# barathanaslan/whisper-ipa

Measured on AMD Instinct MI355X. Metric: audio-seconds/sec transcribed (whisper-small, 30s clips), higher is better.
Workload: dtype bf16

## Files before the change

### include/wipa.h

```cpp
#ifndef WIPA_H
#define WIPA_H
#include <stddef.h>
#include <stdint.h>
#ifdef __cplusplus
extern "C" {
#endif

typedef void* wipa_stream_t;

enum { WIPA_F32 = 0, WIPA_BF16 = 1, WIPA_FP8_E4M3 = 2  };
enum { WIPA_OK = 0, WIPA_ERR_ARG = -1, WIPA_ERR_HIP = -2, WIPA_ERR_STATE = -3 };

#define WIPA_N_SAMPLES 480000
#define WIPA_N_FRAMES 3000
#define WIPA_N_FFT 400
#define WIPA_HOP 160
#define WIPA_HEAD_DIM 64

int wipa_version(void);
const char* wipa_last_error(void);

int wipa_stream_create(wipa_stream_t* out);
int wipa_stream_create_cu_limited(int n_cus, wipa_stream_t* out);
int wipa_stream_destroy(wipa_stream_t s);
// ... 76 lines not shown
                   const float* b, int rows, int D, float eps, wipa_stream_t s);

int wipa_layernorm_fp8(const float* x, int64_t ldx, void* y, int64_t ldy, float* y_scale, const float* w, const float* b, int rows,
                       int D, float eps, wipa_stream_t s);
int wipa_rowquant_fp8(const void* x, int x_dtype, int64_t ldx, void* y, int64_t ldy, float* y_scale, int rows, int D, wipa_stream_t s);

int wipa_add_slabs_layernorm(float* x, int64_t ldx, const float* slabs, int n_slabs, int64_t slab_stride, void* y,
                             int y_dtype, int64_t ldy, const float* w, const float* b, int rows, int D, float eps,
                             wipa_stream_t s);

int wipa_embed_tokens(const int32_t* tokens, int64_t ld_tok, int B, int T, int t_start, const int32_t* pos_dev,
                      const void* tok_emb, int emb_dtype, const float* emb_scale, const float* pos_emb, float* x, int D,
                      wipa_stream_t s);

typedef struct wipa_attn_desc {
    const void* q;
    const void* k;
    const void* v;
    void* out;
    const int32_t* tk_dev;
    const int32_t* q_row_dev;
    float* lse;
    int64_t q_bs, q_rs, q_hs;
    int64_t k_bs, k_rs, k_hs;
    int64_t v_bs, v_rs, v_hs;
    int64_t o_bs, o_rs, o_hs;
    int32_t B, H, Tq, Tk;
    int32_t causal, dtype;
} wipa_attn_desc;
int wipa_attention(const wipa_attn_desc* d, wipa_stream_t s);

int wipa_flash_attn_enc_bf16(const void* qk, int64_t ldqk, const void* vt, int64_t ldvt, void* out, int64_t ldo,
                             int B, int H, int T, wipa_stream_t s);
int wipa_flash_attn_enc_f32(const float* q, int64_t ldq, const float* k, int64_t ldk, const float* v, int64_t ldv, float* out,
                            int64_t ldo, int B, int H, int T, int f32_split, wipa_stream_t s);

int wipa_decode_attn(const wipa_attn_desc* d, wipa_stream_t s);
int wipa_decode_cross_attn(const void* q, const void* kv, void* out, int B, int H, int Tk, int dtype,
                           wipa_stream_t s);
int wipa_decode_cross_attn_multi(const void* q, const void* kv, void* out, int B, int H, int Tk, int n_q, int dtype,
                                 wipa_stream_t s);

int wipa_decode_cross_attn_grouped(const void* q, const void* kv, void* out, int B, int H, int Tk, int n_q, int n_group, int dtype,
                                   wipa_stream_t s);

typedef struct wipa_self_block_desc {
    const float* x;
    const float* ln_w;
    const float* ln_b;
    const void* wqkv;
    const float* bqkv;
    const void* wo;
    void* kcache;
    void* vcache;
    const int32_t* pos;
    float* slabs;
    int64_t kv_batch_stride, slab_stride;
    int32_t B, d, H, dtype;
    float eps, qk_scale;
} wipa_self_block_desc;
int wipa_decode_self_block(const wipa_self_block_desc* d, wipa_stream_t s);
typedef struct wipa_cross_block_desc {
    const float* x_in;
    float* x_out;
    const float* slabs;
    const float* bias_o;
// ... 298 lines not shown
```

### whisper_ipa_amd/_lib.py

```python
from __future__ import annotations

import ctypes as C
import os
import threading

_HERE = os.path.dirname(os.path.abspath(__file__))
LIB_PATH = os.path.join(_HERE, "libwipa.so")

WIPA_F32, WIPA_BF16, WIPA_FP8_E4M3 = 0, 1, 2
GREEDY_PARTS = 2048
RESAMPLE_TILE = 512
SCORE_MAX_LEN = 1024
ENC_GLOBAL, ENC_PER_LAYER = 7, 14
DEC_GLOBAL, DEC_PER_LAYER, DEC_FP8_PER_LAYER = 4, 20, 6
GEMM_DISPATCH = ("tile128", "tile256", "tile384", "tile384n", "tile256p", "skinny", "skinny_fp8", "skinny_ln", "kmajor", "split_k",
                 "tile_fp8", "tile_fp8_384")
ENC_FP8_PER_LAYER = 8
DEC_ABSORBED_PER_LAYER = 1

c_void_p, c_int, c_int64, c_size_t, c_float = C.c_void_p, C.c_int, C.c_int64, C.c_size_t, C.c_float


class GemmDesc(C.Structure):
    _fields_ = [
# ... 67 lines not shown
    _fields_ = [(n, c_int64) for n in (
        "total_bytes", "tokens", "ld_tok", "pos", "not_done", "sum_logprobs", "logits", "ld_logits",
        "cross_kv", "self_kv", "scratch")]


_P = C.POINTER
SIGNATURES = {
    "wipa_version": (c_int, []),
    "wipa_last_error": (C.c_char_p, []),
    "wipa_stream_create": (c_int, [C.POINTER(c_void_p)]),
    "wipa_stream_create_cu_limited": (c_int, [c_int, C.POINTER(c_void_p)]),
    "wipa_stream_destroy": (c_int, [c_void_p]),
    "wipa_resample_pad": (c_int, [c_void_p, c_size_t, c_void_p, _P(PcmClipDesc), c_int, c_void_p, c_size_t, c_void_p, c_void_p]),
    "wipa_logmel_tables_bytes": (c_size_t, [c_int]),
    "wipa_logmel_init": (c_int, [c_void_p, c_int, c_void_p]),
    "wipa_logmel_workspace_bytes": (c_size_t, [c_int, c_int]),
    "wipa_logmel": (c_int, [c_void_p, c_int, c_int, c_void_p, c_void_p, c_int, c_void_p, c_size_t, c_void_p]),
    "wipa_mel_pad_cast": (c_int, [c_void_p, c_int, c_int, c_void_p, c_int, c_void_p]),
    "wipa_gemm": (c_int, [_P(GemmDesc), c_void_p]),
    "wipa_gemm_dispatch_counts": (c_int, [_P(c_int64), c_int, c_int]),
    "wipa_layernorm": (c_int, [c_void_p, c_int, c_int64, c_void_p, c_int, c_int64, c_void_p, c_void_p, c_int, c_int,
                               c_float, c_void_p]),
    "wipa_layernorm_fp8": (c_int, [c_void_p, c_int64, c_void_p, c_int64, c_void_p, c_void_p, c_void_p, c_int, c_int, c_float, c_void_p]),
    "wipa_rowquant_fp8": (c_int, [c_void_p, c_int, c_int64, c_void_p, c_int64, c_void_p, c_int, c_int, c_void_p]),
    "wipa_add_slabs_layernorm": (c_int, [c_void_p, c_int64, c_void_p, c_int, c_int64, c_void_p, c_int, c_int64, c_void_p,
                                         c_void_p, c_int, c_int, c_float, c_void_p]),
    "wipa_embed_tokens": (c_int, [c_void_p, c_int64, c_int, c_int, c_int, c_void_p, c_void_p, c_int, c_void_p, c_void_p, c_void_p,
                                  c_int, c_void_p]),
    "wipa_attention": (c_int, [_P(AttnDesc), c_void_p]),
    "wipa_flash_attn_enc_f32": (c_int, [c_void_p, c_int64, c_void_p, c_int64, c_void_p, c_int64, c_void_p, c_int64, c_int, c_int,
                                       c_int, c_int, c_void_p]),
    "wipa_flash_attn_enc_bf16": (c_int, [c_void_p, c_int64, c_void_p, c_int64, c_void_p, c_int64, c_int, c_int, c_int,
                                         c_void_p]),
    "wipa_decode_attn": (c_int, [_P(AttnDesc), c_void_p]),
    "wipa_decode_cross_attn": (c_int, [c_void_p, c_void_p, c_void_p, c_int, c_int, c_int, c_int, c_void_p]),
    "wipa_decode_self_block": (c_int, [_P(SelfBlockDesc), c_void_p]),
    "wipa_decode_cross_block": (c_int, [_P(CrossBlockDesc), c_void_p]),
    "wipa_cross_absorbed_splits": (c_int, [c_int, c_int]),
    "wipa_cross_absorbed_resident_groups_for": (c_int, [c_int, c_int, c_int, c_int, c_int64]),
    "wipa_cross_absorbed_resident_groups": (c_int, [c_int, c_int, c_int, c_int]),
    "wipa_cross_absorbed_scratch_bytes": (c_size_t, [c_int, c_int, c_int]),
    "wipa_cross_absorbed_init": (c_int, [c_int]),
    "wipa_cross_absorbed_attention": (c_int, [c_void_p, c_int64, c_void_p, c_void_p, c_void_p, c_void_p, c_void_p, c_int64, c_void_p, c_size_t,
                                              c_int, c_int, c_int, c_int, c_float, c_int, c_void_p]),
    "wipa_cross_absorbed_stream": (c_int, [c_void_p, c_void_p, c_size_t, c_int, c_int, c_int, c_int, c_int, c_void_p]),
    "wipa_decode_cross_absorbed_block": (c_int, [_P(CrossBlockDesc), c_void_p, c_void_p, c_void_p, c_void_p, c_size_t, c_void_p]),
    "wipa_decode_cross_absorbed_block_out": (c_int, [_P(CrossBlockDesc), c_void_p, c_void_p, c_void_p, c_void_p, c_void_p, c_void_p, c_int64,
                                                     c_void_p, c_size_t, c_void_p]),
    "wipa_greedy_step": (c_int, [c_void_p, c_int64, c_int, c_int, c_void_p, c_void_p, c_void_p, c_int64, c_void_p, c_int,
                                 c_int, c_void_p, c_void_p, c_void_p]),
    "wipa_add_i32": (c_int, [c_void_p, C.c_int32, c_void_p]),
    "wipa_greedy_step_embed": (c_int, [c_void_p, c_int64, c_int, c_int, c_void_p, c_void_p, c_void_p, c_int64, c_void_p, c_void_p, c_void_p,
                                       c_int, c_int, c_void_p, c_void_p, c_void_p, c_int, c_void_p, c_void_p, c_int, c_void_p, c_void_p,
                                       c_void_p, c_void_p, c_int, c_int, c_float, c_void_p]),
    "wipa_timestamp_step": (c_int, [c_void_p, c_int64, c_int, c_int, c_void_p, c_void_p, c_void_p, c_int64, c_void_p, c_int, c_int,
                                    _P(DecodeRules), c_void_p, c_void_p, c_void_p]),
    "wipa_timestamp_step_embed": (c_int, [c_void_p, c_int64, c_int, c_int, c_void_p, c_void_p, c_void_p, c_int64, c_void_p, c_void_p, c_void_p,
                                          c_int, c_int, _P(DecodeRules), c_void_p, c_void_p, c_void_p, c_int, c_void_p, c_void_p, c_int,
                                          c_void_p, c_void_p, c_void_p, c_void_p, c_int, c_int, c_float, c_void_p]),
    "wipa_sample_record_bytes": (c_size_t, [c_int]),
    "wipa_sample_record_fill": (c_int, [c_void_p, c_size_t, C.c_uint64, c_int, c_float, c_void_p, c_int]),
    "wipa_sample_step": (c_int, [c_void_p, c_int64, c_int, c_int, c_void_p, c_void_p, c_void_p, c_int64, c_void_p, c_int, c_int,
                                 _P(DecodeRules), c_void_p, c_void_p, c_void_p, c_void_p]),
    "wipa_sample_step_embed": (c_int, [c_void_p, c_int64, c_int, c_int, c_void_p, c_void_p, c_void_p, c_int64, c_void_p, c_void_p, c_void_p,
                                       c_int, c_int, _P(DecodeRules), c_void_p, c_void_p, c_void_p, c_void_p, c_int, c_void_p, c_void_p, c_int,
                                       c_void_p, c_void_p, c_void_p, c_void_p, c_int, c_int, c_float, c_void_p]),
# ... 155 lines not shown
```

### whisper_ipa_amd/csrc/attention.hip

```cpp
#include <cstring>

#include "attn_stream.h"
#include "wipa_common.h"

namespace {

struct AttnParams {
    const char* q;
    const char* k;
    const char* v;
    char* out;
    const int32_t* tk_dev;
    const int32_t* q_row_dev;
    float* lse;
    int64_t q_bs, q_rs, q_hs, k_bs, k_rs, k_hs, v_bs, v_rs, v_hs, o_bs, o_rs, o_hs;
    int Tq, Tk, causal, H;
};

template <bool RAGGED, bool GROUPED = false, bool BEAM = false>
struct AttnArgs : AttnParams {};
template <>
struct AttnArgs<true> : AttnParams {
    const int32_t* k_start;
};
// ... 383 lines not shown
                    const int key = kt * 64 + 32 * u + (i & 3) + 8 * (i >> 2) + 4 * hh;            \
                    if (key >= T) S[u][i] = NEG_BIG;                                               \
                }                                                                                  \
        }                                                                                          \
        float mx = NEG_BIG;                                                                        \
        _Pragma("unroll") for (int u = 0; u < 2; ++u)                                              \
            _Pragma("unroll") for (int i = 0; i < 16; ++i) mx = fmaxf(mx, S[u][i]);                \
        mx = fmaxf(mx, __shfl_xor(mx, 32, 64));                                                    \
        const float m_new = fmaxf(m, mx * LOG2E);                                                  \
        f32x2 psum2 = {0.f, 0.f};                                                                  \
        const f32x2 l2e = {LOG2E, LOG2E}, mneg = {-m_new, -m_new};                                 \
        _Pragma("unroll") for (int u = 0; u < 2; ++u)                                              \
            _Pragma("unroll") for (int i = 0; i < 16; i += 2) {                                    \
                const f32x2 x = __builtin_elementwise_fma(f32x2{S[u][i], S[u][i + 1]}, l2e, mneg); \
                const f32x2 pv = {__builtin_amdgcn_exp2f(x.x), __builtin_amdgcn_exp2f(x.y)};       \
                S[u][i] = pv.x;                                                                    \
                S[u][i + 1] = pv.y;                                                                \
                psum2 += pv;                                                                       \
            }                                                                                      \
        const float psum = psum2.x + psum2.y;                                                      \
        if (__any(m_new > m)) {                                                                    \
            const float alpha = __builtin_amdgcn_exp2f(m - m_new);                                 \
            l *= alpha;                                                                            \
            _Pragma("unroll") for (int i = 0; i < 16; ++i) {                                       \
                O[0][i] *= alpha;                                                                  \
                O[1][i] *= alpha;                                                                  \
            }                                                                                      \
            m = m_new;                                                                             \
        }                                                                                          \
        l += psum;                                                                                 \
    } while (0)
#define WIPA_FLASH_SOFTMAX_FINISH() l += __shfl_xor(l, 32, 64)

__global__ __launch_bounds__(512) void flash_enc_bf16_kernel(const __bf16* __restrict__ qk, int64_t ldqk,
                                                             const __bf16* __restrict__ vt, int64_t ldvt,
                                                             __bf16* __restrict__ out, int64_t ldo, int H, int T) {
    __shared__ __attribute__((aligned(16))) char smem[4 * FA_TILE];
    const int tid = threadIdx.x, lane = tid & 63, wave = tid >> 6;
    const int r = lane & 31, hh = lane >> 5;
    const int h = blockIdx.y, b = blockIdx.z;
    const int D = H * 64;
    const int nw = blockDim.x >> 6;
    const int q0 = blockIdx.x * (nw * 32) + wave * 32;
    const int nkt = (T + 63) / 64;

    bf16x8 qf[4];
    {
        const int qrow = min(q0 + r, T - 1);
        const __bf16* qp = qk + ((int64_t)b * T + qrow) * ldqk + h * 64 + 8 * hh;
#pragma unroll
        for (int s = 0; s < 4; ++s) qf[s] = *reinterpret_cast<const bf16x8*>(qp + 16 * s);
    }
    typedef __attribute__((address_space(3))) void* lds_t;
    const __bf16* kbase = qk + (int64_t)b * T * ldqk + D + h * 64;
    const __bf16* vbase = vt + ((int64_t)b * D + h * 64) * ldvt;
    const __amdgpu_buffer_rsrc_t rK = __builtin_amdgcn_make_buffer_rsrc((void*)kbase, 0, (int)(((int64_t)(T - 1) * ldqk + 64) * 2), 0x00020000);
    const __amdgpu_buffer_rsrc_t rV = __builtin_amdgcn_make_buffer_rsrc((void*)vbase, 0, (int)(((int64_t)63 * ldvt + ldvt) * 2), 0x00020000);
    const int wv = __builtin_amdgcn_readfirstlane(wave);
    const int ppw = 8 / nw;
    int offK[2], offV[2];
#pragma unroll
    for (int i = 0; i < 2; ++i) {
        const int row = 8 * (ppw * wv + i) + (lane >> 3);
        const int c = (lane & 7) ^ ((row >> 1) & 7);
        offK[i] = row * (int)ldqk * 2 + c * 16;
        offV[i] = row * (int)ldvt * 2 + c * 16;
    }
    auto stage = [&](int kt, int buf) {
        char* base = smem + buf * 2 * FA_TILE + (ppw * wv) * 1024;
        const int k0 = kt * 64;
#pragma unroll
        for (int i = 0; i < 2; ++i) {
            if (i < ppw) {
                __builtin_amdgcn_raw_ptr_buffer_load_lds(rK, (lds_t)(base + i * 1024), 16, offK[i], k0 * (int)ldqk * 2, 0, 0);
                __builtin_amdgcn_raw_ptr_buffer_load_lds(rV, (lds_t)(base + FA_TILE + i * 1024), 16, offV[i], k0 * 2, 0, 0);
            }
        }
    };

    f32x16 O[2];
#pragma unroll
    for (int i = 0; i < 16; ++i) O[0][i] = O[1][i] = 0.f;
    float m = NEG_BIG, l = 0.f;
    const int rsw = (r >> 1) & 7;

    stage(0, 0);
    asm volatile("s_waitcnt vmcnt(0)" ::: "memory");
    __syncthreads();
    for (int kt = 0; kt < nkt; ++kt) {
        if (kt + 1 < nkt) stage(kt + 1, (kt + 1) & 1);
        const char* kbuf = smem + (kt & 1) * 2 * FA_TILE;
        const char* vbuf = kbuf + FA_TILE;
        f32x16 S[2];
#pragma unroll
        for (int u = 0; u < 2; ++u) {
#pragma unroll
            for (int i = 0; i < 16; ++i) S[u][i] = 0.f;
            const char* krow = kbuf + (32 * u + r) * FA_ROWB;
#pragma unroll
            for (int s = 0; s < 4; ++s) {
                const bf16x8 kf = *reinterpret_cast<const bf16x8*>(krow + (((2 * s + hh) ^ rsw) << 4));
                S[u] = __builtin_amdgcn_mfma_f32_32x32x16_bf16(kf, qf[s], S[u], 0, 0, 0);
            }
        }
        WIPA_FLASH_SOFTMAX_TILE();
#pragma unroll
        for (int u = 0; u < 2; ++u)
#pragma unroll
            for (int sp = 0; sp < 2; ++sp) {
                bf16x8 pb;
#pragma unroll
                for (int j = 0; j < 8; ++j) pb[j] = (__bf16)S[u][8 * sp + j];
#pragma unroll
                for (int dt = 0; dt < 2; ++dt) {
                    const char* vrow = vbuf + (32 * dt + r) * FA_ROWB + 8 * hh;
                    const int c0 = 4 * u + 2 * sp;
                    const bf16x4 lo = *reinterpret_cast<const bf16x4*>(vrow + ((c0 ^ rsw) << 4));
                    const bf16x4 hi = *reinterpret_cast<const bf16x4*>(vrow + (((c0 + 1) ^ rsw) << 4));
                    const bf16x8 vf = {lo[0], lo[1], lo[2], lo[3], hi[0], hi[1], hi[2], hi[3]};
                    O[dt] = __builtin_amdgcn_mfma_f32_32x32x16_bf16(vf, pb, O[dt], 0, 0, 0);
                    asm volatile("" ::: "memory");
                }
            }
        asm volatile("s_waitcnt vmcnt(0)" ::: "memory");
        __syncthreads();
    }
    WIPA_FLASH_SOFTMAX_FINISH();
    const int qrow = q0 + r;
    if (qrow < T) {
        const float inv = 1.f / l;
        __bf16* op = out + ((int64_t)b * T + qrow) * ldo + h * 64 + 4 * hh;
#pragma unroll
        for (int dt = 0; dt < 2; ++dt)
#pragma unroll
            for (int g4 = 0; g4 < 4; ++g4) {
                bf16x4 o = {(__bf16)(O[dt][4 * g4] * inv), (__bf16)(O[dt][4 * g4 + 1] * inv),
                            (__bf16)(O[dt][4 * g4 + 2] * inv), (__bf16)(O[dt][4 * g4 + 3] * inv)};
                *reinterpret_cast<bf16x4*>(op + 32 * dt + 8 * g4) = o;
            }
    }
}

constexpr int FF_LD = 68;
constexpr int FF_TILE = 64 * FF_LD;

__device__ __forceinline__ void stage_k_parity(float* krow, int kseg, const f32x4 (&rk)[4]) {
    float* kt = krow + 8 * kseg;
    *reinterpret_cast<f32x4*>(kt) = f32x4{rk[0][0], rk[0][2], rk[1][0], rk[1][2]};
    *reinterpret_cast<f32x4*>(kt + 4) = f32x4{rk[2][0], rk[2][2], rk[3][0], rk[3][2]};
    *reinterpret_cast<f32x4*>(kt + 32) = f32x4{rk[0][1], rk[0][3], rk[1][1], rk[1][3]};
    *reinterpret_cast<f32x4*>(kt + 36) = f32x4{rk[2][1], rk[2][3], rk[3][1], rk[3][3]};
}
__device__ __forceinline__ void stage_k_plain(float* krow, int kseg, const f32x4 (&rk)[4]) {
    float* kt = krow + 16 * kseg;
#pragma unroll
    for (int c = 0; c < 4; ++c) *reinterpret_cast<f32x4*>(kt + 4 * c) = rk[c];
// ... 132 lines not shown
                S[u] = __builtin_amdgcn_mfma_f32_32x32x16_bf16(kh, qh[s], S[u], 0, 0, 0);
            }
        }
        WIPA_FLASH_SOFTMAX_TILE();
#pragma unroll
        for (int u = 0; u < 2; ++u)
#pragma unroll
            for (int sp = 0; sp < 2; ++sp) {
                bf16x8 ph, pl;
                split_bf16x2(f32x4{S[u][8 * sp], S[u][8 * sp + 1], S[u][8 * sp + 2], S[u][8 * sp + 3]},
                             f32x4{S[u][8 * sp + 4], S[u][8 * sp + 5], S[u][8 * sp + 6], S[u][8 * sp + 7]}, ph, pl);
#pragma unroll
                for (int dt = 0; dt < 2; ++dt) {
                    const float* vr = vbuf + (32 * dt + r) * FF_LD + 32 * u + 16 * sp + 4 * hh;
                    bf16x8 vh, vl;
                    split_bf16x2(*reinterpret_cast<const f32x4*>(vr), *reinterpret_cast<const f32x4*>(vr + 8), vh, vl);
                    O[dt] = __builtin_amdgcn_mfma_f32_32x32x16_bf16(vh, pl, O[dt], 0, 0, 0);
                    O[dt] = __builtin_amdgcn_mfma_f32_32x32x16_bf16(vl, ph, O[dt], 0, 0, 0);
                    O[dt] = __builtin_amdgcn_mfma_f32_32x32x16_bf16(vh, ph, O[dt], 0, 0, 0);
                }
            }
        WIPA_FLASH_F32_TILE_END();
    }
    WIPA_FLASH_F32_TAIL();
}

#undef WIPA_FLASH_F32_INDICES
#undef WIPA_FLASH_F32_STAGING
#undef WIPA_FLASH_F32_TILE_BEGIN
#undef WIPA_FLASH_F32_TILE_END
#undef WIPA_FLASH_F32_TAIL
#undef WIPA_FLASH_SOFTMAX_TILE
#undef WIPA_FLASH_SOFTMAX_FINISH

}

static bool attn_strides_aligned(const wipa_attn_desc* d) {
    const int64_t al = d->dtype == WIPA_BF16 ? 8 : 4;
    return d->q_rs % al == 0 && d->k_rs % al == 0 && d->v_rs % al == 0 && d->q_hs % al == 0 && d->k_hs % al == 0 && d->v_hs % al == 0 &&
           d->q_bs % al == 0 && d->k_bs % al == 0 && d->v_bs % al == 0;
}

static void fill_attn_params(const wipa_attn_desc* d, AttnParams& p) {
    p.q = (const char*)d->q;
    p.k = (const char*)d->k;
    p.v = (const char*)d->v;
    p.out = (char*)d->out;
    p.tk_dev = d->tk_dev;
    p.q_row_dev = d->q_row_dev;
    p.lse = d->lse;
    p.q_bs = d->q_bs; p.q_rs = d->q_rs; p.q_hs = d->q_hs;
    p.k_bs = d->k_bs; p.k_rs = d->k_rs; p.k_hs = d->k_hs;
    p.v_bs = d->v_bs; p.v_rs = d->v_rs; p.v_hs = d->v_hs;
    p.o_bs = d->o_bs; p.o_rs = d->o_rs; p.o_hs = d->o_hs;
    p.Tq = d->Tq;
    p.Tk = d->Tk;
    p.causal = d->causal;
    p.H = d->H;
}

extern "C" int wipa_attention(const wipa_attn_desc* d, wipa_stream_t stream) { return wipa_attention_as(d, d ? d->Tq : 0, stream); }

int wipa_attention_as(const wipa_attn_desc* d, int path_tq, wipa_stream_t stream) {
    WIPA_REQUIRE(d && d->q && d->k && d->v && d->out, "wipa_attention: null pointer");
    WIPA_REQUIRE(d->B > 0 && d->H > 0 && d->Tq > 0, "wipa_attention: bad shape");
    WIPA_REQUIRE(d->dtype == WIPA_F32 || d->dtype == WIPA_BF16, "wipa_attention: bad dtype %d", d->dtype);
// ... 14 lines not shown
        hipLaunchKernelGGL((attn_generic_kernel<__bf16>), grid, dim3(256), 0, (hipStream_t)stream, p);
    WIPA_LAUNCH_CHECK();
    return WIPA_OK;
}

extern "C" int wipa_attention_ragged(const wipa_attn_desc* d, const int32_t* starts_dev, wipa_stream_t stream) {
    WIPA_REQUIRE(d && d->q && d->k && d->v && d->out && starts_dev, "wipa_attention_ragged: null pointer (starts_dev is required)");
    WIPA_REQUIRE(d->B > 0 && d->H > 0 && d->Tq > 0, "wipa_attention_ragged: bad shape");
    WIPA_REQUIRE(d->dtype == WIPA_F32 || d->dtype == WIPA_BF16, "wipa_attention_ragged: bad dtype %d", d->dtype);
    WIPA_REQUIRE(attn_strides_aligned(d), "wipa_attention_ragged: strides must keep 16-byte alignment");
    WIPA_REQUIRE(d->causal && d->Tq == d->Tk && !d->tk_dev && !d->q_row_dev && !d->lse,
                 "wipa_attention_ragged: causal self-attention with Tq == Tk (Tq=%d Tk=%d), no device-side offsets, no lse", d->Tq, d->Tk);
    AttnArgs<true> p;
    fill_attn_params(d, p);
    p.k_start = starts_dev;
    dim3 grid((d->Tq + 15) / 16, d->H, d->B);
    if (d->dtype == WIPA_F32)
        hipLaunchKernelGGL((attn_generic_kernel<float, true>), grid, dim3(256), 0, (hipStream_t)stream, p);
    else
        hipLaunchKernelGGL((attn_generic_kernel<__bf16, true>), grid, dim3(256), 0, (hipStream_t)stream, p);
    WIPA_LAUNCH_CHECK();
    return WIPA_OK;
}

extern "C" int wipa_flash_attn_enc_bf16(const void* qk, int64_t ldqk, const void* vt, int64_t ldvt, void* out, int64_t ldo,
                                        int B, int H, int T, wipa_stream_t stream) {
    WIPA_REQUIRE(qk && vt && out, "wipa_flash_attn_enc_bf16: null pointer");
    WIPA_REQUIRE(ldqk % 8 == 0 && ldvt % 8 == 0 && ldo % 4 == 0, "wipa_flash_attn_enc_bf16: ld alignment");
    WIPA_REQUIRE(ldvt >= ((T + 63) / 64) * 64, "wipa_flash_attn_enc_bf16: ldvt=%lld must cover ceil64(T)", (long long)ldvt);
    WIPA_REQUIRE(B > 0 && H > 0 && T > 0, "wipa_flash_attn_enc_bf16: bad shape");
    static const int q128 = [] { const char* e = getenv("WIPA_FLASH_Q128"); return e ? atoi(e) : 0; }();
    const int nw = (T > 256 && !q128) ? 8 : 4;
    dim3 grid((T + nw * 32 - 1) / (nw * 32), H, B);
    hipLaunchKernelGGL(flash_enc_bf16_kernel, grid, dim3(nw * 64), 0, (hipStream_t)stream, (const __bf16*)qk, ldqk,
                       (const __bf16*)vt, ldvt, (__bf16*)out, ldo, H, T);
    WIPA_LAUNCH_CHECK();
    return WIPA_OK;
}

extern "C" int wipa_flash_attn_enc_f32(const float* q, int64_t ldq, const float* k, int64_t ldk, const float* v, int64_t ldv,
                                       float* out, int64_t ldo, int B, int H, int T, int f32_split, wipa_stream_t stream) {
    WIPA_REQUIRE(q && k && v && out, "wipa_flash_attn_enc_f32: null pointer");
    WIPA_REQUIRE(ldq % 4 == 0 && ldk % 4 == 0 && ldv % 4 == 0 && ldo % 4 == 0, "wipa_flash_attn_enc_f32: row strides must be multiples of 4");
    WIPA_REQUIRE(((uintptr_t)q % 16) == 0 && ((uintptr_t)k % 16) == 0 && ((uintptr_t)v % 16) == 0 && ((uintptr_t)out % 16) == 0,
                 "wipa_flash_attn_enc_f32: operands must be 16-byte aligned");
    WIPA_REQUIRE(B > 0 && H > 0 && T > 0, "wipa_flash_attn_enc_f32: bad shape");
    dim3 grid((T + 127) / 128, H, B);
    if (!f32_split)
        hipLaunchKernelGGL(flash_enc_f32_kernel, grid, dim3(256), 0, (hipStream_t)stream, q, ldq, k, ldk, v, ldv, out, ldo, T);
    else
        hipLaunchKernelGGL(flash_enc_f32s_kernel, grid, dim3(256), 0, (hipStream_t)stream, q, ldq, k, ldk, v, ldv, out, ldo, T);
    WIPA_LAUNCH_CHECK();
    return WIPA_OK;
}

extern "C" int wipa_decode_attn(const wipa_attn_desc* d, wipa_stream_t stream) {
    WIPA_REQUIRE(d && d->q && d->k && d->v && d->out, "wipa_decode_attn: null pointer");
    WIPA_REQUIRE(d->B > 0 && d->H > 0 && d->Tq == 1, "wipa_decode_attn: one query row per (b,h) (Tq=%d)", d->Tq);
    WIPA_REQUIRE(d->dtype == WIPA_F32 || d->dtype == WIPA_BF16, "wipa_decode_attn: bad dtype %d", d->dtype);
    WIPA_REQUIRE(attn_strides_aligned(d), "wipa_decode_attn: strides must keep 16-byte alignment");
    AttnArgs<false> p;
    fill_attn_params(d, p);
    const bool short_cache = d->Tk + (d->tk_dev ? 448 : 0) <= 512;
    static const int self_waves = [] { const char* e = getenv("WIPA_SELF_ATTN_WAVES"); return e ? atoi(e) : 4; }();
    if (short_cache && self_waves == 4) {
        dim3 grid(d->H, d->B);
        if (d->dtype == WIPA_F32)
            hipLaunchKernelGGL((decode_attn_kernel<float, 4, false>), grid, dim3(256), 0, (hipStream_t)stream, p);
// ... 146 lines not shown
```

### whisper_ipa_amd/csrc/runtime.hip

```cpp
#include <algorithm>
#include <cstdarg>
#include <cstdlib>
#include <cstring>
#include <strings.h>
#include <map>
#include <mutex>
#include <tuple>
#include <vector>

#include "wipa_common.h"

static thread_local char g_err[512] = "";
void wipa_set_error(const char* fmt, ...) {
    va_list ap;
    va_start(ap, fmt);
    vsnprintf(g_err, sizeof(g_err), fmt, ap);
    va_end(ap);
}
extern "C" const char* wipa_last_error(void) { return g_err; }
extern "C" int wipa_version(void) { return 100; }

extern "C" int wipa_stream_create_cu_limited(int n_cus, wipa_stream_t* out) {
    int dev = 0, total = 0;
    WIPA_CHECK_HIP(hipGetDevice(&dev));
// ... 115 lines not shown
    return c->dec_w_dtype == WIPA_FP8_E4M3 ? (const float*)w[WIPA_DEC_GLOBAL + WIPA_DEC_PER_LAYER * c->n_text_layer] : nullptr;
}

int gemm(const void* A, int64_t lda, const void* W, int64_t ldw, void* C, int64_t ldc, int M, int N, int K, int in_dt,
         int out_dt, const float* bias, int act, const void* residual, wipa_stream_t s, wipa_gemm_desc* extra = nullptr) {
    wipa_gemm_desc g;
    if (extra) g = *extra; else memset(&g, 0, sizeof(g));
    g.A = A; g.lda = lda; g.W = W; g.ldw = ldw; g.C = C; g.ldc = ldc;
    g.M = M; g.N = N; g.K = K; g.in_dtype = in_dt; g.out_dtype = out_dt;
    g.bias = bias; g.act = act; g.residual = residual;
    g.f32_split = t_f32_split;
    if (t_w8) {
        auto it = t_w8->find(W);
        if (it != t_w8->end()) {
            g.w_dtype = WIPA_FP8_E4M3;
            g.w_scale = it->second;
        }
    }
    return wipa_gemm(&g, s);
}

int gemm_f8(const void* A, int64_t lda, const float* a_scale, const void* W, int64_t ldw, const float* w_scale, void* C, int64_t ldc,
            int M, int N, int K, int out_dt, const float* bias, int act, const void* residual, wipa_stream_t s,
            wipa_gemm_desc* extra = nullptr) {
    wipa_gemm_desc g;
    if (extra) g = *extra; else memset(&g, 0, sizeof(g));
    g.A = A; g.lda = lda; g.W = W; g.ldw = ldw; g.C = C; g.ldc = ldc;
    g.M = M; g.N = N; g.K = K; g.in_dtype = WIPA_FP8_E4M3; g.out_dtype = out_dt;
    g.bias = bias; g.act = act; g.residual = residual;
    g.a_scale = a_scale; g.w_scale = w_scale;
    return wipa_gemm(&g, s);
}

struct EncWs {
    size_t c1, x, ln, qk, v, ao, h, total;
};
EncWs enc_ws(const wipa_model_cfg* c, int B) {
    const size_t e = wipa_dtype_size(c->dtype), d = c->n_audio_state, M = (size_t)B * c->n_audio_ctx;
    EncWs w;
    size_t o = 0;
    w.c1 = o; o += align256(((size_t)B * ROWS_IN + 4) * d * e);
    w.x = o;  o += align256(M * d * 4);
    w.ln = o; o += align256(M * d * e);
    w.qk = o; o += align256(M * 2 * d * e);
    w.v = o;  o += align256(c->dtype == WIPA_BF16 ? (size_t)B * d * T_ENC_PAD * e + 256 : M * d * e);
    w.ao = o; o += align256(M * d * e);
    w.h = o;  o += align256(M * 4 * d * e);
    w.total = o;
    return w;
}

}

extern "C" size_t wipa_encoder_workspace_bytes(const wipa_model_cfg* cfg, int B) {
    if (!cfg || B <= 0) return 0;
    return enc_ws(cfg, B).total;
}

extern "C" int wipa_encoder_forward(const wipa_model_cfg* cfg, const void* const* w, const void* mel_padded, void* out,
                                    void* workspace, size_t workspace_bytes, int B, wipa_stream_t stream) {
    RT_CALL(cfg_check(cfg));
    SplitScope split_scope(cfg);
    WIPA_REQUIRE(w && mel_padded && out && workspace && B > 0, "wipa_encoder_forward: null pointer / bad batch");
    const EncWs L = enc_ws(cfg, B);
    WIPA_REQUIRE(workspace_bytes >= L.total, "wipa_encoder_forward: workspace too small (%zu < %zu)", workspace_bytes, L.total);
    hipStream_t s = (hipStream_t)stream;
    const int dt = cfg->dtype;
    const size_t e = wipa_dtype_size(dt);
    const int d = cfg->n_audio_state, H = cfg->n_audio_head, T = cfg->n_audio_ctx, M = B * T;
    char* ws = (char*)workspace;
    void* c1 = ws + L.c1;
    float* x = (float*)(ws + L.x);
    void* ln = ws + L.ln;
    void* qk = ws + L.qk;
    void* vb = ws + L.v;
    void* ao = ws + L.ao;
    void* hb = ws + L.h;
    const int K1 = round_up(3 * cfg->n_mels, k_multiple(dt));

    WIPA_CHECK_HIP(hipMemsetAsync(c1, 0, (size_t)d * e, s));
    {
        wipa_gemm_desc g;
        memset(&g, 0, sizeof(g));
        g.rg_in = ROWS_IN; g.rg_valid = WIPA_N_FRAMES; g.rg_stride = (int64_t)ROWS_IN * d; g.zero_invalid_rows = 1;
        g.c_offset = d;
        PROF(PROF_GEMM, gemm(mel_padded, cfg->n_mels, w[0], K1, c1, d, B * ROWS_IN, d, K1, dt, dt, (const float*)w[1], 1, nullptr,
                     stream, &g));
    }
    {
        wipa_gemm_desc g;
        memset(&g, 0, sizeof(g));
        g.rg_in = T + 1; g.rg_valid = T; g.rg_stride = (int64_t)T * d;
        g.pos = (const float*)w[4]; g.ldpos = d;
        PROF(PROF_GEMM, gemm(c1, 2 * d, w[2], 3 * d, x, d, B * (T + 1), d, 3 * d, dt, WIPA_F32, (const float*)w[3], 1, nullptr,
                     stream, &g));
    }
    if (dt == WIPA_BF16) WIPA_CHECK_HIP(hipMemsetAsync(vb, 0, (size_t)B * d * T_ENC_PAD * e, s));
    const bool f8 = cfg->enc_act_fp8 != 0;
    float* ln_scale = (float*)((char*)ln + (size_t)M * d);
    const void* const* w8 = w + WIPA_ENC_GLOBAL + WIPA_ENC_PER_LAYER * cfg->n_audio_layer;
    for (int l = 0; l < cfg->n_audio_layer; ++l) {
        const void* const* lw = w + WIPA_ENC_GLOBAL + WIPA_ENC_PER_LAYER * l;
        const void* const* l8 = w8 + WIPA_ENC_FP8_PER_LAYER * l;
        if (f8) PROF(PROF_NORM, wipa_layernorm_fp8(x, d, ln, d, ln_scale, (const float*)lw[0], (const float*)lw[1], M, d, 1e-5f, stream));
        else PROF(PROF_NORM, wipa_layernorm(x, WIPA_F32, d, ln, dt, d, (const float*)lw[0], (const float*)lw[1], M, d, 1e-5f, stream));
        {
            wipa_gemm_desc g;
            memset(&g, 0, sizeof(g));
            g.col_scale_n = 2 * d; g.col_scale = QK_SCALE;
            if (f8) PROF(PROF_GEMM, gemm_f8(ln, d, ln_scale, l8[0], d, (const float*)l8[1], qk, 2 * d, M, 2 * d, d, dt, (const float*)lw[3], 0,
                                            nullptr, stream, &g));
            else PROF(PROF_GEMM, gemm(ln, d, lw[2], d, qk, 2 * d, M, 2 * d, d, dt, dt, (const float*)lw[3], 0, nullptr, stream, &g));
        }
        if (dt == WIPA_BF16) {
            wipa_gemm_desc g;
            memset(&g, 0, sizeof(g));
            g.bias_along_m = 1; g.cg_in = T; g.cg_stride = (int64_t)d * T_ENC_PAD;
            if (f8) PROF(PROF_GEMM, gemm_f8(l8[2], d, (const float*)l8[3], ln, d, ln_scale, vb, T_ENC_PAD, d, M, d, dt, (const float*)lw[5], 0,
                                            nullptr, stream, &g));
            else PROF(PROF_GEMM, gemm(lw[4], d, ln, d, vb, T_ENC_PAD, d, M, d, dt, dt, (const float*)lw[5], 0, nullptr, stream, &g));
            PROF(PROF_ATTN, wipa_flash_attn_enc_bf16(qk, 2 * d, vb, T_ENC_PAD, ao, d, B, H, T, stream));
        } else {
            PROF(PROF_GEMM, gemm(ln, d, lw[4], d, vb, d, M, d, d, dt, dt, (const float*)lw[5], 0, nullptr, stream));
            PROF(PROF_ATTN, wipa_flash_attn_enc_f32((const float*)qk, 2 * d, (const float*)qk + d, 2 * d, (const float*)vb, d, (float*)ao, d,
                                            B, H, T, t_f32_split, stream));
        }
        PROF(PROF_GEMM, gemm(ao, d, lw[6], d, x, d, M, d, d, dt, WIPA_F32, (const float*)lw[7], 0, x, stream));
        if (f8) {
            PROF(PROF_NORM, wipa_layernorm_fp8(x, d, ln, d, ln_scale, (const float*)lw[8], (const float*)lw[9], M, d, 1e-5f, stream));
            PROF(PROF_GEMM, gemm_f8(ln, d, ln_scale, l8[4], d, (const float*)l8[5], hb, 4 * d, M, 4 * d, d, dt, (const float*)lw[11], 1, nullptr,
                                    stream));
            void* h8 = qk;
            float* h_scale = (float*)ao;
            PROF(PROF_NORM, wipa_rowquant_fp8(hb, dt, 4 * d, h8, 4 * d, h_scale, M, 4 * d, stream));
            PROF(PROF_GEMM, gemm_f8(h8, 4 * d, h_scale, l8[6], 4 * d, (const float*)l8[7], x, d, M, d, 4 * d, WIPA_F32, (const float*)lw[13], 0,
                                    x, stream));
        } else {
            PROF(PROF_NORM, wipa_layernorm(x, WIPA_F32, d, ln, dt, d, (const float*)lw[8], (const float*)lw[9], M, d, 1e-5f, stream));
            PROF(PROF_GEMM, gemm(ln, d, lw[10], d, hb, 4 * d, M, 4 * d, d, dt, dt, (const float*)lw[11], 1, nullptr, stream));
            PROF(PROF_GEMM, gemm(hb, 4 * d, lw[12], 4 * d, x, d, M, d, 4 * d, dt, WIPA_F32, (const float*)lw[13], 0, x, stream));
        }
    }
    PROF(PROF_NORM, wipa_layernorm(x, WIPA_F32, d, out, dt, d, (const float*)w[5], (const float*)w[6], M, d, 1e-5f, stream));
    return WIPA_OK;
}

namespace {
// ... 1668 lines not shown
```

### whisper_ipa_amd/ops.py

```python
from __future__ import annotations

import ctypes as C
from typing import Optional

import torch

from . import _lib
from .runtime import dt_code, on_stream, ptr, sptr


def gemm(A: torch.Tensor, W: torch.Tensor, C_out: torch.Tensor, *, M: int, N: int, K: int, lda: int, ldw: int, ldc: int,
         bias: Optional[torch.Tensor] = None, bias_along_m: bool = False, act: int = 0,
         residual: Optional[torch.Tensor] = None, pos: Optional[torch.Tensor] = None, ldpos: int = 0,
         col_scale_n: int = 0, col_scale: float = 1.0, rg_in: int = 0, rg_valid: int = 0, rg_stride: int = 0,
         cg_in: int = 0, cg_stride: int = 0, c_offset: int = 0, c_offset_dev: Optional[torch.Tensor] = None,
         zero_invalid_rows: bool = False, k_slices: int = 0, slab_stride: int = 0, f32_split: bool = False,
         a_trans: bool = False, w_trans: bool = False) -> torch.Tensor:
    L = _lib.lib()
    d = _lib.GemmDesc()
    d.A, d.W, d.C = ptr(A), ptr(W), ptr(C_out)
    d.bias, d.residual, d.pos, d.c_offset_dev = ptr(bias), ptr(residual), ptr(pos), ptr(c_offset_dev)
    d.lda, d.ldw, d.ldc, d.ldpos = lda, ldw, ldc, ldpos
    d.rg_stride, d.cg_stride, d.c_offset = rg_stride, cg_stride, c_offset
    d.M, d.N, d.K = M, N, K
# ... 105 lines not shown
        _lib.check(L.wipa_attention(C.byref(d), sptr(s)), "wipa_attention")
    return out


def decode_attn(q: torch.Tensor, k: torch.Tensor, v: torch.Tensor, Tk: Optional[int] = None,
                tk_dev: Optional[torch.Tensor] = None, q_row_dev: Optional[torch.Tensor] = None) -> torch.Tensor:
    L = _lib.lib()
    B, _, H, hd = q.shape
    assert hd == 64
    with on_stream() as s:
        out = torch.empty(B, H, 64, dtype=q.dtype, device=q.device)
        d = _lib.AttnDesc()
        d.q, d.k, d.v, d.out = ptr(q), ptr(k), ptr(v), ptr(out)
        d.tk_dev, d.q_row_dev = ptr(tk_dev), ptr(q_row_dev)
        d.q_bs, d.q_rs, d.q_hs = q.stride(0), q.stride(1), q.stride(2)
        d.k_bs, d.k_rs, d.k_hs = k.stride(0), k.stride(1), k.stride(2)
        d.v_bs, d.v_rs, d.v_hs = v.stride(0), v.stride(1), v.stride(2)
        d.o_bs, d.o_rs, d.o_hs = out.stride(0), out.stride(0), out.stride(1)
        d.B, d.H, d.Tq, d.Tk, d.causal, d.dtype = B, H, 1, (k.shape[1] if Tk is None else Tk), 0, dt_code(q.dtype)
        _lib.check(L.wipa_decode_attn(C.byref(d), sptr(s)), "wipa_decode_attn")
    return out


def flash_attn_enc(qk: torch.Tensor, vt: torch.Tensor, B: int, H: int, T: int) -> torch.Tensor:
    L = _lib.lib()
    D = H * 64
    with on_stream() as s:
        out = torch.empty(B * T, D, dtype=torch.bfloat16, device=qk.device)
        _lib.check(L.wipa_flash_attn_enc_bf16(ptr(qk), qk.stride(0), ptr(vt), vt.stride(1), ptr(out), D, B, H, T, sptr(s)),
                   "wipa_flash_attn_enc_bf16")
    return out


def flash_attn_enc_f32(qk: torch.Tensor, v: torch.Tensor, B: int, H: int, T: int, f32_split: bool = False) -> torch.Tensor:
    L = _lib.lib()
    D = H * 64
    assert qk.dtype == torch.float32 and v.dtype == torch.float32
    with on_stream() as s:
        out = torch.empty(B * T, D, dtype=torch.float32, device=qk.device)
        k = qk[:, D:]
        _lib.check(L.wipa_flash_attn_enc_f32(ptr(qk), qk.stride(0), ptr(k), qk.stride(0), ptr(v), v.stride(0), ptr(out), D,
                                             B, H, T, int(f32_split), sptr(s)), "wipa_flash_attn_enc_f32")
    return out


def decode_cross_attn(q: torch.Tensor, kv: torch.Tensor) -> torch.Tensor:
    L = _lib.lib()
    B, twoH, Tk, hd = kv.shape
    assert hd == 64 and kv.is_contiguous() and q.is_contiguous()
    with on_stream() as s:
        out = torch.empty_like(q)
        _lib.check(L.wipa_decode_cross_attn(ptr(q), ptr(kv), ptr(out), B, twoH // 2, Tk, dt_code(q.dtype), sptr(s)),
                   "wipa_decode_cross_attn")
    return out


def embed_tokens(tokens: torch.Tensor, tok_emb: torch.Tensor, pos_emb: torch.Tensor, t_start: int = 0) -> torch.Tensor:
    L = _lib.lib()
    B, T = tokens.shape
    D = tok_emb.shape[1]
    with on_stream() as s:
        x = torch.empty(B * T, D, dtype=torch.float32, device=tok_emb.device)
        _lib.check(L.wipa_embed_tokens(ptr(tokens), tokens.stride(0), B, T, t_start, None, ptr(tok_emb), dt_code(tok_emb.dtype),
                                       None, ptr(pos_emb), ptr(x), D, sptr(s)), "wipa_embed_tokens")
    return x

# ... 12 lines not shown
```

Baseline: 27610.

## Keep encoder V row-major and transpose in LDS with ds_read_tr in flash attention

Adds a row-major-V variant of the bf16 encoder flash-attention kernel. V fragments are transposed on the fly via ds_read_b64_tr_b16 LDS reads, pipelined with the PV MFMAs. The encoder now runs the V projection as a plain GEMM writing row-major output, which removes the transposed, padded V layout and its per-forward memset. The variant is on by default for bf16 without fp8 activations. It adds inline-asm waitcnt sequencing and swizzle addressing that must exactly match the staging layout.

New measurement: 27690 (median of 6 runs). About the same (+0.3%).

```diff
diff --git a/include/wipa.h b/include/wipa.h
--- a/include/wipa.h
+++ b/include/wipa.h
@@ -132,6 +132,8 @@
 
 int wipa_flash_attn_enc_bf16(const void* qk, int64_t ldqk, const void* vt, int64_t ldvt, void* out, int64_t ldo,
                              int B, int H, int T, wipa_stream_t s);
+int wipa_flash_attn_enc_bf16_rowv(const void* qk, int64_t ldqk, const void* v, int64_t ldv, void* out, int64_t ldo,
+                                  int B, int H, int T, wipa_stream_t s);
 int wipa_flash_attn_enc_f32(const float* q, int64_t ldq, const float* k, int64_t ldk, const float* v, int64_t ldv, float* out,
                             int64_t ldo, int B, int H, int T, int f32_split, wipa_stream_t s);
 
diff --git a/whisper_ipa_amd/_lib.py b/whisper_ipa_amd/_lib.py
--- a/whisper_ipa_amd/_lib.py
+++ b/whisper_ipa_amd/_lib.py
@@ -123,6 +123,8 @@
                                        c_int, c_int, c_void_p]),
     "wipa_flash_attn_enc_bf16": (c_int, [c_void_p, c_int64, c_void_p, c_int64, c_void_p, c_int64, c_int, c_int, c_int,
                                          c_void_p]),
+    "wipa_flash_attn_enc_bf16_rowv": (c_int, [c_void_p, c_int64, c_void_p, c_int64, c_void_p, c_int64, c_int, c_int, c_int,
+                                              c_void_p]),
     "wipa_decode_attn": (c_int, [_P(AttnDesc), c_void_p]),
     "wipa_decode_cross_attn": (c_int, [c_void_p, c_void_p, c_void_p, c_int, c_int, c_int, c_int, c_void_p]),
     "wipa_decode_self_block": (c_int, [_P(SelfBlockDesc), c_void_p]),
diff --git a/whisper_ipa_amd/csrc/attention.hip b/whisper_ipa_amd/csrc/attention.hip
--- a/whisper_ipa_amd/csrc/attention.hip
+++ b/whisper_ipa_amd/csrc/attention.hip
@@ -439,6 +439,22 @@
     } while (0)
 #define WIPA_FLASH_SOFTMAX_FINISH() l += __shfl_xor(l, 32, 64)
 
+#define WIPA_FA_TR4_ISSUE(Y, A, IMM)                                                                                      \
+    asm volatile("ds_read_b64_tr_b16 %0, %4 offset:" #IMM "\n\tds_read_b64_tr_b16 %1, %5 offset:" #IMM                    \
+                 "\n\tds_read_b64_tr_b16 %2, %6 offset:" #IMM "\n\tds_read_b64_tr_b16 %3, %7 offset:" #IMM                \
+                 : "=&v"(Y[0]), "=&v"(Y[1]), "=&v"(Y[2]), "=&v"(Y[3])                                                     \
+                 : "v"(A[0]), "v"(A[1]), "v"(A[2]), "v"(A[3])                                                             \
+                 : "memory")
+#define WIPA_FA_TR4_NEXT(Y, X, A, IMM)                                                                                    \
+    asm volatile("ds_read_b64_tr_b16 %0, %8 offset:" #IMM "\n\tds_read_b64_tr_b16 %1, %9 offset:" #IMM                    \
+                 "\n\tds_read_b64_tr_b16 %2, %10 offset:" #IMM "\n\tds_read_b64_tr_b16 %3, %11 offset:" #IMM              \
+                 "\n\ts_waitcnt lgkmcnt(4)"                                                                               \
+                 : "=&v"(Y[0]), "=&v"(Y[1]), "=&v"(Y[2]), "=&v"(Y[3]), "+v"(X[0]), "+v"(X[1]), "+v"(X[2]), "+v"(X[3])     \
+                 : "v"(A[0]), "v"(A[1]), "v"(A[2]), "v"(A[3])                                                             \
+                 : "memory")
+#define WIPA_FA_TR4_LAST(X) asm volatile("s_waitcnt lgkmcnt(0)" : "+v"(X[0]), "+v"(X[1]), "+v"(X[2]), "+v"(X[3]) : : "memory")
+
+template <bool VROW>
 __global__ __launch_bounds__(512) void flash_enc_bf16_kernel(const __bf16* __restrict__ qk, int64_t ldqk,
                                                              const __bf16* __restrict__ vt, int64_t ldvt,
                                                              __bf16* __restrict__ out, int64_t ldo, int H, int T) {
@@ -460,9 +476,10 @@
     }
     typedef __attribute__((address_space(3))) void* lds_t;
     const __bf16* kbase = qk + (int64_t)b * T * ldqk + D + h * 64;
-    const __bf16* vbase = vt + ((int64_t)b * D + h * 64) * ldvt;
+    const __bf16* vbase = VROW ? vt + (int64_t)b * T * ldvt + h * 64 : vt + ((int64_t)b * D + h * 64) * ldvt;
     const __amdgpu_buffer_rsrc_t rK = __builtin_amdgcn_make_buffer_rsrc((void*)kbase, 0, (int)(((int64_t)(T - 1) * ldqk + 64) * 2), 0x00020000);
-    const __amdgpu_buffer_rsrc_t rV = __builtin_amdgcn_make_buffer_rsrc((void*)vbase, 0, (int)(((int64_t)63 * ldvt + ldvt) * 2), 0x00020000);
+    const __amdgpu_buffer_rsrc_t rV = __builtin_amdgcn_make_buffer_rsrc(
+        (void*)vbase, 0, (int)((VROW ? (int64_t)(T - 1) * ldvt + 64 : (int64_t)63 * ldvt + ldvt) * 2), 0x00020000);
     const int wv = __builtin_amdgcn_readfirstlane(wave);
     const int ppw = 8 / nw;
     int offK[2], offV[2];
@@ -480,7 +497,8 @@
         for (int i = 0; i < 2; ++i) {
             if (i < ppw) {
                 __builtin_amdgcn_raw_ptr_buffer_load_lds(rK, (lds_t)(base + i * 1024), 16, offK[i], k0 * (int)ldqk * 2, 0, 0);
-                __builtin_amdgcn_raw_ptr_buffer_load_lds(rV, (lds_t)(base + FA_TILE + i * 1024), 16, offV[i], k0 * 2, 0, 0);
+                __builtin_amdgcn_raw_ptr_buffer_load_lds(rV, (lds_t)(base + FA_TILE + i * 1024), 16, offV[i],
+                                                         VROW ? k0 * (int)ldvt * 2 : k0 * 2, 0, 0);
             }
         }
     };
@@ -490,6 +508,16 @@
     for (int i = 0; i < 16; ++i) O[0][i] = O[1][i] = 0.f;
     float m = NEG_BIG, l = 0.f;
     const int rsw = (r >> 1) & 7;
+    unsigned tv[4];
+    if constexpr (VROW) {
+        const int q = (r & 15) >> 2, p = r & 3;
+#pragma unroll
+        for (int i = 0; i < 4; ++i) {
+            const int row = 4 * hh + 8 * (i & 1) + q;
+            const int ch = 4 * (i >> 1) + 2 * (r >> 4) + (p >> 1);
+            tv[i] = (unsigned)(uintptr_t)(lds_t)smem + FA_TILE + row * FA_ROWB + ((ch ^ ((row >> 1) & 7)) << 4) + 8 * (p & 1);
+        }
+    }
 
     stage(0, 0);
     asm volatile("s_waitcnt vmcnt(0)" ::: "memory");
@@ -511,6 +539,33 @@
             }
         }
         WIPA_FLASH_SOFTMAX_TILE();
+        if constexpr (VROW) {
+            typedef int v2i32 __attribute__((ext_vector_type(2)));
+            typedef int v4i32x __attribute__((ext_vector_type(4)));
+            v2i32 xe[4], xo[4];
+#define WIPA_FA_PV(U, SP, X)                                                                                              \
+    {                                                                                                                     \
+        bf16x8 pb;                                                                                                        \
+        _Pragma("unroll") for (int j = 0; j < 8; ++j) pb[j] = (__bf16)S[U][8 * SP + j];                                   \
+        _Pragma("unroll") for (int dt = 0; dt < 2; ++dt) {                                                                \
+            const bf16x8 vf = __builtin_bit_cast(bf16x8, v4i32x{X[2 * dt][0], X[2 * dt][1], X[2 * dt + 1][0], X[2 * dt + 1][1]}); \
+            O[dt] = __builtin_amdgcn_mfma_f32_32x32x16_bf16(vf, pb, O[dt], 0, 0, 0);                                      \
+        }                                                                                                                 \
+    }
+            WIPA_FA_TR4_ISSUE(xe, tv, 0);
+            WIPA_FA_TR4_NEXT(xo, xe, tv, 2048);
+            WIPA_FA_PV(0, 0, xe)
+            WIPA_FA_TR4_NEXT(xe, xo, tv, 4096);
+            WIPA_FA_PV(0, 1, xo)
+            WIPA_FA_TR4_NEXT(xo, xe, tv, 6144);
+            WIPA_FA_PV(1, 0, xe)
+            WIPA_FA_TR4_LAST(xo);
+            WIPA_FA_PV(1, 1, xo)
+#undef WIPA_FA_PV
+            const int other = (kt & 1) ? -2 * FA_TILE : 2 * FA_TILE;
+#pragma unroll
+            for (int i = 0; i < 4; ++i) tv[i] += other;
+        } else {
 #pragma unroll
         for (int u = 0; u < 2; ++u)
 #pragma unroll
@@ -529,6 +584,7 @@
                     asm volatile("" ::: "memory");
                 }
             }
+        }
         asm volatile("s_waitcnt vmcnt(0)" ::: "memory");
         __syncthreads();
     }
@@ -727,6 +783,9 @@
 #undef WIPA_FLASH_F32_TAIL
 #undef WIPA_FLASH_SOFTMAX_TILE
 #undef WIPA_FLASH_SOFTMAX_FINISH
+#undef WIPA_FA_TR4_ISSUE
+#undef WIPA_FA_TR4_NEXT
+#undef WIPA_FA_TR4_LAST
 
 }
 
@@ -807,8 +866,25 @@
     static const int q128 = [] { const char* e = getenv("WIPA_FLASH_Q128"); return e ? atoi(e) : 0; }();
     const int nw = (T > 256 && !q128) ? 8 : 4;
     dim3 grid((T + nw * 32 - 1) / (nw * 32), H, B);
-    hipLaunchKernelGGL(flash_enc_bf16_kernel, grid, dim3(nw * 64), 0, (hipStream_t)stream, (const __bf16*)qk, ldqk,
+    hipLaunchKernelGGL(flash_enc_bf16_kernel<false>, grid, dim3(nw * 64), 0, (hipStream_t)stream, (const __bf16*)qk, ldqk,
                        (const __bf16*)vt, ldvt, (__bf16*)out, ldo, H, T);
+    WIPA_LAUNCH_CHECK();
+    return WIPA_OK;
+}
+
+extern "C" int wipa_flash_attn_enc_bf16_rowv(const void* qk, int64_t ldqk, const void* v, int64_t ldv, void* out, int64_t ldo,
+                                             int B, int H, int T, wipa_stream_t stream) {
+    WIPA_REQUIRE(qk && v && out, "wipa_flash_attn_enc_bf16_rowv: null pointer");
+    WIPA_REQUIRE(ldqk % 8 == 0 && ldv % 8 == 0 && ldo % 4 == 0 && ((uintptr_t)qk % 16) == 0 && ((uintptr_t)v % 16) == 0,
+                 "wipa_flash_attn_enc_bf16_rowv: ld / pointer alignment");
+    WIPA_REQUIRE(B > 0 && H > 0 && T > 0, "wipa_flash_attn_enc_bf16_rowv: bad shape");
+    WIPA_REQUIRE(((int64_t)T + 64) * 2 * (ldqk > ldv ? ldqk : ldv) < ((int64_t)1 << 31),
+                 "wipa_flash_attn_enc_bf16_rowv: a clip's rows must span less than 2 GiB");
+    static const int q128 = [] { const char* e = getenv("WIPA_FLASH_Q128"); return e ? atoi(e) : 0; }();
+    const int nw = (T > 256 && !q128) ? 8 : 4;
+    dim3 grid((T + nw * 32 - 1) / (nw * 32), H, B);
+    hipLaunchKernelGGL(flash_enc_bf16_kernel<true>, grid, dim3(nw * 64), 0, (hipStream_t)stream, (const __bf16*)qk, ldqk,
+                       (const __bf16*)v, ldv, (__bf16*)out, ldo, H, T);
     WIPA_LAUNCH_CHECK();
     return WIPA_OK;
 }
diff --git a/whisper_ipa_amd/csrc/runtime.hip b/whisper_ipa_amd/csrc/runtime.hip
--- a/whisper_ipa_amd/csrc/runtime.hip
+++ b/whisper_ipa_amd/csrc/runtime.hip
@@ -171,18 +171,23 @@
     return wipa_gemm(&g, s);
 }
 
+bool enc_v_row_major(const wipa_model_cfg* c) {
+    static const bool on = [] { const char* e = getenv("WIPA_ENC_QKV"); return !(e && atoi(e) == 0); }();
+    return on && c->dtype == WIPA_BF16 && !c->enc_act_fp8;
+}
 struct EncWs {
     size_t c1, x, ln, qk, v, ao, h, total;
 };
 EncWs enc_ws(const wipa_model_cfg* c, int B) {
     const size_t e = wipa_dtype_size(c->dtype), d = c->n_audio_state, M = (size_t)B * c->n_audio_ctx;
+    const bool vrow = enc_v_row_major(c);
     EncWs w;
     size_t o = 0;
     w.c1 = o; o += align256(((size_t)B * ROWS_IN + 4) * d * e);
     w.x = o;  o += align256(M * d * 4);
     w.ln = o; o += align256(M * d * e);
     w.qk = o; o += align256(M * 2 * d * e);
-    w.v = o;  o += align256(c->dtype == WIPA_BF16 ? (size_t)B * d * T_ENC_PAD * e + 256 : M * d * e);
+    w.v = o;  o += align256(c->dtype == WIPA_BF16 && !vrow ? (size_t)B * d * T_ENC_PAD * e + 256 : M * d * e);
     w.ao = o; o += align256(M * d * e);
     w.h = o;  o += align256(M * 4 * d * e);
     w.total = o;
@@ -234,7 +239,8 @@
         PROF(PROF_GEMM, gemm(c1, 2 * d, w[2], 3 * d, x, d, B * (T + 1), d, 3 * d, dt, WIPA_F32, (const float*)w[3], 1, nullptr,
                      stream, &g));
     }
-    if (dt == WIPA_BF16) WIPA_CHECK_HIP(hipMemsetAsync(vb, 0, (size_t)B * d * T_ENC_PAD * e, s));
+    const bool vrow = enc_v_row_major(cfg);
+    if (dt == WIPA_BF16 && !vrow) WIPA_CHECK_HIP(hipMemsetAsync(vb, 0, (size_t)B * d * T_ENC_PAD * e, s));
     const bool f8 = cfg->enc_act_fp8 != 0;
     float* ln_scale = (float*)((char*)ln + (size_t)M * d);
     const void* const* w8 = w + WIPA_ENC_GLOBAL + WIPA_ENC_PER_LAYER * cfg->n_audio_layer;
@@ -251,7 +257,10 @@
                                             nullptr, stream, &g));
             else PROF(PROF_GEMM, gemm(ln, d, lw[2], d, qk, 2 * d, M, 2 * d, d, dt, dt, (const float*)lw[3], 0, nullptr, stream, &g));
         }
-        if (dt == WIPA_BF16) {
+        if (vrow) {
+            PROF(PROF_GEMM, gemm(ln, d, lw[4], d, vb, d, M, d, d, dt, dt, (const float*)lw[5], 0, nullptr, stream));
+            PROF(PROF_ATTN, wipa_flash_attn_enc_bf16_rowv(qk, 2 * d, vb, d, ao, d, B, H, T, stream));
+        } else if (dt == WIPA_BF16) {
             wipa_gemm_desc g;
             memset(&g, 0, sizeof(g));
             g.bias_along_m = 1; g.cg_in = T; g.cg_stride = (int64_t)d * T_ENC_PAD;
diff --git a/whisper_ipa_amd/ops.py b/whisper_ipa_amd/ops.py
--- a/whisper_ipa_amd/ops.py
+++ b/whisper_ipa_amd/ops.py
@@ -161,6 +161,18 @@
     return out
 
 
+def flash_attn_enc_rowv(qk: torch.Tensor, v: torch.Tensor, B: int, H: int, T: int) -> torch.Tensor:
+    L = _lib.lib()
+    D = H * 64
+    assert qk.dtype == torch.bfloat16 and v.dtype == torch.bfloat16 and qk.stride(1) == 1 and v.stride(1) == 1
+    assert qk.shape[1] >= 2 * D and v.shape[1] >= D
+    with on_stream() as s:
+        out = torch.empty(B * T, D, dtype=torch.bfloat16, device=qk.device)
+        _lib.check(L.wipa_flash_attn_enc_bf16_rowv(ptr(qk), qk.stride(0), ptr(v), v.stride(0), ptr(out), D, B, H, T, sptr(s)),
+                   "wipa_flash_attn_enc_bf16_rowv")
+    return out
+
+
 def flash_attn_enc_f32(qk: torch.Tensor, v: torch.Tensor, B: int, H: int, T: int, f32_split: bool = False) -> torch.Tensor:
     L = _lib.lib()
     D = H * 64
```
